# isl-org/Open3D-PointNet2-Semantic3D

Hardware: AMD Instinct MI355X
Metric: points/sec through SA+FP stack (B=16,N=8192) (higher is better)
Workload: dtype f32

## Files before the change

open3d-pointnet2-semantic3d_amd/csrc/pn2_interpolate.hip:

```cpp
#include <math.h>

#include "pn2_common.h"
#include "pn2_three_nn.h"

namespace {

using namespace pn2nn;

PN2_TUNABLE(int, g_nn_blocks, 2048)

template <int kNnChunks>
__global__ void __launch_bounds__(kNnThreads)
three_nn_kernel(int n, int m, const float* __restrict__ xyz1_all, int ld1,
                const float* __restrict__ xyz2_all, float* __restrict__ dist_all,
                int* __restrict__ idx_all) {
    __shared__ __attribute__((aligned(16))) unsigned char slds[kNnWaves * kNnWaveLdsBytes];
    const int wave = __builtin_amdgcn_readfirstlane(threadIdx.x >> 6);
    const int bi = blockIdx.y;
    three_nn_wave<kNnChunks>(n, m, xyz1_all + (size_t)bi * n * ld1, xyz2_all + (size_t)bi * m * 3, dist_all + (size_t)bi * n * 3,
                             idx_all + (size_t)bi * n * 3, blockIdx.x * kNnWaves + wave, gridDim.x * kNnWaves,
                             nn_wave_lds(slds, wave), ld1);
}

template <typename VT, int VEC>
__global__ void __launch_bounds__(256)
three_interpolate_kernel(int m, int c, int n, const float* __restrict__ points_all,
                         const int* __restrict__ idx_all, const float* __restrict__ weight_all,
                         float* __restrict__ out_all) {
    const unsigned cv = (unsigned)c / VEC;
    const unsigned total = (unsigned)n * cv;
    const int bi = blockIdx.y;
    const VT* __restrict__ pts = reinterpret_cast<const VT*>(points_all + (size_t)bi * m * c);
    const int* __restrict__ idx = idx_all + (size_t)bi * n * 3;
    const float* __restrict__ w = weight_all + (size_t)bi * n * 3;
    VT* __restrict__ out = reinterpret_cast<VT*>(out_all + (size_t)bi * n * c);
    for (unsigned e = blockIdx.x * blockDim.x + threadIdx.x; e < total; e += gridDim.x * blockDim.x) {
        const unsigned row = e / cv, col = e - row * cv;
        const int i1 = idx[row * 3 + 0], i2 = idx[row * 3 + 1], i3 = idx[row * 3 + 2];
        const float w1 = w[row * 3 + 0], w2 = w[row * 3 + 1], w3 = w[row * 3 + 2];
        const VT p1 = pts[(size_t)i1 * cv + col], p2 = pts[(size_t)i2 * cv + col], p3 = pts[(size_t)i3 * cv + col];
        out[e] = (p1 * w1 + p2 * w2) + p3 * w3;
    }
}

template <typename VT, int VEC>
__global__ void __launch_bounds__(256)
three_interpolate_grad_kernel(int n, int c, int m, const float* __restrict__ grad_out_all,
                              const int* __restrict__ idx_all, const float* __restrict__ weight_all,
                              float* __restrict__ grad_points_all) {
    const unsigned cv = (unsigned)c / VEC;
    const unsigned total = (unsigned)n * cv;
    const int bi = blockIdx.y;
    const VT* __restrict__ go = reinterpret_cast<const VT*>(grad_out_all + (size_t)bi * n * c);
    const int* __restrict__ idx = idx_all + (size_t)bi * n * 3;
    const float* __restrict__ w = weight_all + (size_t)bi * n * 3;
    float* __restrict__ gp = grad_points_all + (size_t)bi * m * c;
    for (unsigned e = blockIdx.x * blockDim.x + threadIdx.x; e < total; e += gridDim.x * blockDim.x) {
        const unsigned row = e / cv, col = e - row * cv;
        const VT g = go[e];
#pragma unroll
        for (int t = 0; t < 3; ++t) {
            const int ii = idx[row * 3 + t];
            const float wt = w[row * 3 + t];
            float* dst = gp + (size_t)ii * c + col * VEC;
            if constexpr (VEC == 4) {
                atomicAdd(dst + 0, g.x * wt); atomicAdd(dst + 1, g.y * wt);
                atomicAdd(dst + 2, g.z * wt); atomicAdd(dst + 3, g.w * wt);
            } else {
                atomicAdd(dst, g * wt);
            }
        }
    }
}

__global__ void __launch_bounds__(256)
ti_csr_count_kernel(int n3, int m, const int* __restrict__ idx_all, int* __restrict__ cnt_all) {
    const int bi = blockIdx.y;
    const int* __restrict__ idx = idx_all + (size_t)bi * n3;
    int* __restrict__ cnt = cnt_all + (size_t)bi * m;
    for (int e = blockIdx.x * blockDim.x + threadIdx.x; e < n3; e += gridDim.x * blockDim.x) atomicAdd(&cnt[idx[e]], 1);
}

__global__ void __launch_bounds__(256)
ti_csr_scan_kernel(int m, int* __restrict__ cnt_all, int* __restrict__ off_all) {
    __shared__ int part[256];
    const int bi = blockIdx.x, t = threadIdx.x;
    int* __restrict__ cnt = cnt_all + (size_t)bi * m;
    int* __restrict__ off = off_all + (size_t)bi * m;
    const int per = (m + 255) / 256;
    const int lo = t * per < m ? t * per : m, hi = lo + per < m ? lo + per : m;
    int sum = 0;
    for (int i = lo; i < hi; ++i) sum += cnt[i];
    part[t] = sum;
    __syncthreads();
    for (int d = 1; d < 256; d <<= 1) {
        const int v = t >= d ? part[t - d] : 0;
        __syncthreads();
        part[t] += v;
        __syncthreads();
    }
    int run = part[t] - sum;
    for (int i = lo; i < hi; ++i) {
        const int v = cnt[i];
        off[i] = run;
        cnt[i] = 0;
        run += v;
    }
}

__global__ void __launch_bounds__(256)
ti_csr_fill_kernel(int n3, int m, int div, const int* __restrict__ idx_all, const float* __restrict__ weight_all,
                   int weight_kind, const int* __restrict__ off_all, int* __restrict__ cur_all, int* __restrict__ ent_q_all,
                   float* __restrict__ ent_w_all) {
    const int bi = blockIdx.y;
    const int* __restrict__ idx = idx_all + (size_t)bi * n3;
    const float* __restrict__ w = weight_all ? weight_all + (size_t)bi * n3 : nullptr;
    const int* __restrict__ off = off_all + (size_t)bi * m;
    int* __restrict__ cur = cur_all + (size_t)bi * m;
    int* __restrict__ eq = ent_q_all + (size_t)bi * n3;
    float* __restrict__ ew = ent_w_all + (size_t)bi * n3;
    for (int e = blockIdx.x * blockDim.x + threadIdx.x; e < n3; e += gridDim.x * blockDim.x) {
        const int s = idx[e];
        const int p = off[s] + atomicAdd(&cur[s], 1);
        eq[p] = e / div;
        float wt = 1.f;
        if (w && weight_kind == 2) {
            const int r = e / 3, j = e - 3 * r;
            const float r1 = 1.0f / fmaxf(w[r * 3 + 0], 1e-10f), r2 = 1.0f / fmaxf(w[r * 3 + 1], 1e-10f);
            const float r3 = 1.0f / fmaxf(w[r * 3 + 2], 1e-10f);
            const float norm = (r1 + r2) + r3;
            wt = (j == 0 ? r1 : (j == 1 ? r2 : r3)) / norm;
        } else if (w) {
            wt = w[e];
        }
        ew[p] = wt;
    }
}

typedef float f32x4_u __attribute__((ext_vector_type(4), aligned(4)));
template <bool ALIGNED>
__device__ __forceinline__ void ti_csr_gather_body(int bx, int bi, int n, int n3, int c, int stride, int m,
                                                   const float* __restrict__ grad_out_all, const int* __restrict__ off_all,
                                                   const int* __restrict__ ent_q_all, const float* __restrict__ ent_w_all,
                                                   float* __restrict__ grad_points_all, int ostride) {
    const int cv = c >> 2;
    const int spb = 256 / cv;
    const int slot = (int)threadIdx.x / cv, col = (int)threadIdx.x - slot * cv;
    const int s = bx * spb + slot;
    if (slot >= spb || s >= m) return;
    const float* __restrict__ gbase = grad_out_all + (size_t)bi * n * stride + 4 * col;
    auto row4 = [&](int q) -> f32x4 {
        if constexpr (ALIGNED) return *reinterpret_cast<const f32x4*>(gbase + (size_t)q * stride);
        else return *reinterpret_cast<const f32x4_u*>(gbase + (size_t)q * stride);
    };
    const int* __restrict__ off = off_all + (size_t)bi * m;
    const int* __restrict__ eq = ent_q_all + (size_t)bi * n3;
    const float* __restrict__ ew = ent_w_all + (size_t)bi * n3;
    const int lo = off[s], hi = s + 1 < m ? off[s + 1] : n3;
    f32x4 acc = {0.f, 0.f, 0.f, 0.f};
    int e = lo;
    for (; e + 3 < hi; e += 4) {
        int q[4]; float w[4]; f32x4 g[4];
#pragma unroll
        for (int u = 0; u < 4; ++u) { q[u] = eq[e + u]; w[u] = ew[e + u]; }
#pragma unroll
        for (int u = 0; u < 4; ++u) g[u] = row4(q[u]);
#pragma unroll
        for (int u = 0; u < 4; ++u) {
            acc.x = __builtin_fmaf(g[u].x, w[u], acc.x); acc.y = __builtin_fmaf(g[u].y, w[u], acc.y);
            acc.z = __builtin_fmaf(g[u].z, w[u], acc.z); acc.w = __builtin_fmaf(g[u].w, w[u], acc.w);
        }
    }
    for (; e < hi; ++e) {
        const f32x4 g = row4(eq[e]);
        const float w = ew[e];
        acc.x = __builtin_fmaf(g.x, w, acc.x); acc.y = __builtin_fmaf(g.y, w, acc.y);
        acc.z = __builtin_fmaf(g.z, w, acc.z); acc.w = __builtin_fmaf(g.w, w, acc.w);
    }
    reinterpret_cast<f32x4*>(grad_points_all + ((size_t)bi * m + s) * ostride)[col] = acc;
}

template <bool ALIGNED>
__global__ void __launch_bounds__(256)
ti_csr_gather_kernel(int n, int n3, int c, int stride, int m, const float* __restrict__ grad_out_all, const int* __restrict__ off_all,
                     const int* __restrict__ ent_q_all, const float* __restrict__ ent_w_all,
                     float* __restrict__ grad_points_all) {
    ti_csr_gather_body<ALIGNED>((int)blockIdx.x, (int)blockIdx.y, n, n3, c, stride, m, grad_out_all, off_all, ent_q_all, ent_w_all,
                                grad_points_all, c);
}

__global__ void __launch_bounds__(256)
fp_interp_concat_kernel(int n, int m, int c1, int c2, int ostride, int rpw, const float* __restrict__ dist_all,
                        const int* __restrict__ idx_all, const float* __restrict__ points1_all,
                        const float* __restrict__ points2_all, float* __restrict__ out_all) {
    const int lane = threadIdx.x & 63;
    const int wave = __builtin_amdgcn_readfirstlane(threadIdx.x >> 6);
    const int bi = blockIdx.y;
    const int cw = ostride;
    const float* __restrict__ dist = dist_all + (size_t)bi * n * 3;
    const int* __restrict__ idx = idx_all + (size_t)bi * n * 3;
    const float* __restrict__ p2 = points2_all + (size_t)bi * m * c2;
    const float* __restrict__ p1 = points1_all ? points1_all + (size_t)bi * n * c1 : nullptr;
    float* __restrict__ out = out_all + (size_t)bi * n * cw;
    for (int row0 = (blockIdx.x * 4 + wave) * rpw; row0 < n; row0 += gridDim.x * 4 * rpw) {
        int r = row0 + (lane < rpw ? lane : rpw - 1);
        r = r < n ? r : n - 1;
        const float d1 = fmaxf(dist[r * 3 + 0], 1e-10f);
        const float d2 = fmaxf(dist[r * 3 + 1], 1e-10f);
        const float d3 = fmaxf(dist[r * 3 + 2], 1e-10f);
        const float r1 = 1.0f / d1, r2 = 1.0f / d2, r3 = 1.0f / d3;
        const float norm = (r1 + r2) + r3;
        const float w1 = r1 / norm, w2 = r2 / norm, w3 = r3 / norm;
        const int i1 = idx[r * 3 + 0], i2 = idx[r * 3 + 1], i3 = idx[r * 3 + 2];
        const int nrows = n - row0 < rpw ? n - row0 : rpw;
        auto one_row = [&](int rr) {
            const float a1 = __uint_as_float(__builtin_amdgcn_readlane(__float_as_uint(w1), rr));
            const float a2 = __uint_as_float(__builtin_amdgcn_readlane(__float_as_uint(w2), rr));
            const float a3 = __uint_as_float(__builtin_amdgcn_readlane(__float_as_uint(w3), rr));
            const float* __restrict__ s1 = p2 + (size_t)__builtin_amdgcn_readlane(i1, rr) * c2;
            const float* __restrict__ s2 = p2 + (size_t)__builtin_amdgcn_readlane(i2, rr) * c2;
            const float* __restrict__ s3 = p2 + (size_t)__builtin_amdgcn_readlane(i3, rr) * c2;
            float* __restrict__ o = out + (size_t)(row0 + rr) * cw;
#pragma unroll 4
            for (int ch = lane; ch < c2; ch += 64) o[ch] = (s1[ch] * a1 + s2[ch] * a2) + s3[ch] * a3;
            if (p1) {
                const float* __restrict__ q = p1 + (size_t)(row0 + rr) * c1;
                for (int ch = lane; ch < c1; ch += 64) o[c2 + ch] = q[ch];
            }
            if (lane < cw - c1 - c2) o[c1 + c2 + lane] = 0.f;
        };
        int rr = 0;
        for (; rr + 1 < nrows; rr += 2) { one_row(rr); one_row(rr + 1); }
        if (rr < nrows) one_row(rr);
    }
}

template <int CHW, int R>
__global__ void __launch_bounds__(256)
fp_interp_concat_rows_kernel(int n, int m, int c1, int c2, int ostride, int rpw, const float* __restrict__ dist_all,
                             const int* __restrict__ idx_all, const float* __restrict__ points1_all,
                             const float* __restrict__ points2_all, float* __restrict__ out_all) {
    const int lane = threadIdx.x & 63;
    const int wave = __builtin_amdgcn_readfirstlane(threadIdx.x >> 6);
    int bx = blockIdx.x, bi = blockIdx.y;
    {
        const unsigned nwg = gridDim.x * gridDim.y;
        if ((nwg & 7u) == 0u) {
            const unsigned lin = blockIdx.x + gridDim.x * blockIdx.y;
            const unsigned swz = (lin & 7u) * (nwg >> 3) + (lin >> 3);
            bx = (int)(swz % gridDim.x);
            bi = (int)(swz / gridDim.x);
        }
    }
    const int cw = ostride;
    const float* __restrict__ dist = dist_all + (size_t)bi * n * 3;
    const int* __restrict__ idx = idx_all + (size_t)bi * n * 3;
    const float* __restrict__ p2 = points2_all + (size_t)bi * m * c2;
    const float* __restrict__ p1 = points1_all ? points1_all + (size_t)bi * n * c1 : p2;
    float* __restrict__ out = out_all + (size_t)bi * n * cw;
    const int c1m = c1 > 0 ? c1 - 1 : 0;
    for (int row0 = (bx * 4 + wave) * rpw; row0 < n; row0 += gridDim.x * 4 * rpw) {
        int r = row0 + (lane < rpw ? lane : rpw - 1);
        r = r < n ? r : n - 1;
        const float d1 = fmaxf(dist[r * 3 + 0], 1e-10f);
        const float d2 = fmaxf(dist[r * 3 + 1], 1e-10f);
        const float d3 = fmaxf(dist[r * 3 + 2], 1e-10f);
        const float r1 = 1.0f / d1, r2 = 1.0f / d2, r3 = 1.0f / d3;
        const float norm = (r1 + r2) + r3;
        const float w1 = r1 / norm, w2 = r2 / norm, w3 = r3 / norm;
        const int i1 = idx[r * 3 + 0], i2 = idx[r * 3 + 1], i3 = idx[r * 3 + 2];
        const int nrows = n - row0 < rpw ? n - row0 : rpw;
        for (int rr = 0; rr < nrows; rr += R) {
            float v[R][CHW];
#pragma unroll
            for (int q = 0; q < R; ++q) {
                const int rx = rr + q < nrows ? rr + q : nrows - 1;
                const float a1 = __uint_as_float(__builtin_amdgcn_readlane(__float_as_uint(w1), rx));
                const float a2 = __uint_as_float(__builtin_amdgcn_readlane(__float_as_uint(w2), rx));
                const float a3 = __uint_as_float(__builtin_amdgcn_readlane(__float_as_uint(w3), rx));
                const float* __restrict__ s1 = p2 + (size_t)__builtin_amdgcn_readlane(i1, rx) * c2;
                const float* __restrict__ s2 = p2 + (size_t)__builtin_amdgcn_readlane(i2, rx) * c2;
                const float* __restrict__ s3 = p2 + (size_t)__builtin_amdgcn_readlane(i3, rx) * c2;
                const float* __restrict__ qp = p1 + (size_t)(row0 + rx) * c1;
#pragma unroll
                for (int j = 0; j < CHW; ++j) {
                    const int col = lane + 64 * j;
                    const int cc = col < c2 ? col : c2 - 1;
                    int ci = col - c2;
                    ci = ci < 0 ? 0 : (ci > c1m ? c1m : ci);
                    const float x1 = s1[cc], x2 = s2[cc], x3 = s3[cc], xp = qp[ci];
                    const float val = (x1 * a1 + x2 * a2) + x3 * a3;
                    v[q][j] = col < c2 ? val : (col < c2 + c1 ? xp : 0.f);
                }
            }
#pragma unroll
            for (int q = 0; q < R; ++q) {
                if (rr + q < nrows) {
                    float* __restrict__ o = out + (size_t)(row0 + rr + q) * cw;
#pragma unroll
                    for (int j = 0; j < CHW; ++j) {
                        const int col = lane + 64 * j;
                        if (col < cw) o[col] = v[q][j];
                    }
                }
            }
        }
    }
}

template <bool P1V>
__global__ void __launch_bounds__(256)
fp_interp_concat_v4_kernel(int n, int m, int c1, int c2, int ostride, int rpw, int sh2, int sht,
                           const float* __restrict__ dist_all, const int* __restrict__ idx_all,
                           const float* __restrict__ points1_all, const float* __restrict__ points2_all,
                           float* __restrict__ out_all) {
    __shared__ __attribute__((aligned(16))) float swt[4 * 64 * 8];
    const int lane = threadIdx.x & 63;
    const int wave = __builtin_amdgcn_readfirstlane(threadIdx.x >> 6);
    int bx = blockIdx.x, bi = blockIdx.y;
    {
        const unsigned nwg = gridDim.x * gridDim.y;
        if ((nwg & 7u) == 0u) {
            const unsigned lin = blockIdx.x + gridDim.x * blockIdx.y;
            const unsigned swz = (lin & 7u) * (nwg >> 3) + (lin >> 3);
            bx = (int)(swz % gridDim.x);
            bi = (int)(swz / gridDim.x);
        }
    }
    const int cv = ostride >> 2, c2v = c2 >> 2;
    const float* __restrict__ dist = dist_all + (size_t)bi * n * 3;
    const int* __restrict__ idx = idx_all + (size_t)bi * n * 3;
    const f32x4* __restrict__ p2 = reinterpret_cast<const f32x4*>(points2_all + (size_t)bi * m * c2);
    const float* __restrict__ p1 = points1_all ? points1_all + (size_t)bi * n * c1 : nullptr;
    f32x4* __restrict__ out = reinterpret_cast<f32x4*>(out_all + (size_t)bi * n * ostride);
    float* wv = swt + wave * 64 * 8;
    const unsigned m2 = (1u << sh2) - 1u, mt = (1u << sht) - 1u;
    for (int row0 = (bx * 4 + wave) * rpw; row0 < n; row0 += gridDim.x * 4 * rpw) {
        {
            int r = row0 + (lane < rpw ? lane : rpw - 1);
            r = r < n ? r : n - 1;
            const float d1 = fmaxf(dist[r * 3 + 0], 1e-10f);
            const float d2 = fmaxf(dist[r * 3 + 1], 1e-10f);
            const float d3 = fmaxf(dist[r * 3 + 2], 1e-10f);
            const float r1 = 1.0f / d1, r2 = 1.0f / d2, r3 = 1.0f / d3;
            const float norm = (r1 + r2) + r3;
            const f32x4 wq = {r1 / norm, r2 / norm, r3 / norm, 0.f};
            const f32x4 iq = {__int_as_float(idx[r * 3 + 0]), __int_as_float(idx[r * 3 + 1]),
                              __int_as_float(idx[r * 3 + 2]), 0.f};
            *reinterpret_cast<f32x4*>(wv + lane * 8) = wq;
            *reinterpret_cast<f32x4*>(wv + lane * 8 + 4) = iq;
        }
        const int nrows = n - row0 < rpw ? n - row0 : rpw;
        const unsigned E = (unsigned)nrows << sh2;
        for (unsigned e0 = lane; e0 < E; e0 += 64 * 4) {
            f32x4 v[4];
#pragma unroll
            for (int u = 0; u < 4; ++u) {
                unsigned e = e0 + 64 * u;
                e = e < E ? e : E - 1;
                const unsigned row = e >> sh2, col = e & m2;
                const f32x4 wq = *reinterpret_cast<const f32x4*>(wv + row * 8);
                const f32x4 iq = *reinterpret_cast<const f32x4*>(wv + row * 8 + 4);
                const f32x4 x1 = p2[(size_t)__float_as_int(iq[0]) * c2v + col];
                const f32x4 x2 = p2[(size_t)__float_as_int(iq[1]) * c2v + col];
                const f32x4 x3 = p2[(size_t)__float_as_int(iq[2]) * c2v + col];
                v[u] = (x1 * wq[0] + x2 * wq[1]) + x3 * wq[2];
            }
#pragma unroll
            for (int u = 0; u < 4; ++u) {
                const unsigned e = e0 + 64 * u;
                if (e < E) out[(size_t)(row0 + (e >> sh2)) * cv + (e & m2)] = v[u];
            }
        }
        const unsigned ET = (unsigned)nrows << sht;
        for (unsigned e = lane; e < ET; e += 64) {
            const unsigned row = e >> sht, ct = e & mt;
            f32x4 t = {0.f, 0.f, 0.f, 0.f};
            if constexpr (P1V) {
                if ((int)ct * 4 < c1) t = *reinterpret_cast<const f32x4*>(p1 + (size_t)(row0 + row) * c1 + ct * 4);
            } else {
#pragma unroll
                for (int i = 0; i < 4; ++i) {
                    const int ch = (int)ct * 4 + i;
                    if (ch < c1) t[i] = p1[(size_t)(row0 + row) * c1 + ch];
                }
            }
            out[(size_t)(row0 + row) * cv + c2v + ct] = t;
        }
    }
}

inline int grid_x_for(unsigned long long total, int block, int batches) {
    unsigned long long g = (total + block - 1) / block;
    unsigned long long cap = (256ull * 8 + batches - 1) / batches;
    if (cap < 1) cap = 1;
    if (g > cap) g = cap;
    if (g < 1) g = 1;
    return (int)g;
}

}

#ifdef PN2_TUNING_HOOKS
extern "C" int pn2_debug_set_interp(int what, int value) { if (what == 12) { g_nn_blocks = value; return 0; } return -1; }
#endif

extern "C" int pn2_three_nn_ld(int b, int n, int m, const float* xyz1, int ld1, const float* xyz2, float* dist,
                               int* idx, void* stream) {
    if (b <= 0 || n <= 0 || m < 3 || ld1 < 3) return PN2_EINVAL;
    if (!xyz1 || !xyz2 || !dist || !idx) return PN2_ENULL;
    if ((long long)n * ld1 > 0x7fffffffLL || (long long)m * 3 > 0x7fffffffLL || b > 65535) return PN2_ERANGE;
    const int blocks_all = (n + kNnWaves * kNnQ - 1) / (kNnWaves * kNnQ);
    int per = (b * blocks_all + g_nn_blocks - 1) / g_nn_blocks;
    if (per < 1) per = 1;
    dim3 grid((blocks_all + per - 1) / per, b);
    hipStream_t st = static_cast<hipStream_t>(stream);
    if (m <= 64) three_nn_kernel<1><<<grid, kNnThreads, 0, st>>>(n, m, xyz1, ld1, xyz2, dist, idx);
    else if (m <= 256) three_nn_kernel<4><<<grid, kNnThreads, 0, st>>>(n, m, xyz1, ld1, xyz2, dist, idx);
    else three_nn_kernel<16><<<grid, kNnThreads, 0, st>>>(n, m, xyz1, ld1, xyz2, dist, idx);
    PN2_RETURN_IF_LAUNCH_FAILED();
    return PN2_OK;
}

extern "C" int pn2_three_nn(int b, int n, int m, const float* xyz1, const float* xyz2, float* dist,
                            int* idx, void* stream) {
    return pn2_three_nn_ld(b, n, m, xyz1, 3, xyz2, dist, idx, stream);
}

extern "C" int pn2_three_interpolate(int b, int m, int c, int n, const float* points, const int* idx,
                                     const float* weight, float* out, void* stream) {
    if (b <= 0 || m <= 0 || c <= 0 || n <= 0) return PN2_EINVAL;
    if (!points || !idx || !weight || !out) return PN2_ENULL;
    if ((unsigned long long)n * c > 0xffffffffull || b > 65535) return PN2_ERANGE;
    hipStream_t st = static_cast<hipStream_t>(stream);
    const bool vec4 = (c % 4 == 0) && (((uintptr_t)points | (uintptr_t)out) % 16 == 0);
    if (vec4) {
        dim3 grid(grid_x_for((unsigned long long)n * (c / 4), 256, b), b);
        three_interpolate_kernel<f32x4, 4><<<grid, 256, 0, st>>>(m, c, n, points, idx, weight, out);
    } else {
        dim3 grid(grid_x_for((unsigned long long)n * c, 256, b), b);
        three_interpolate_kernel<float, 1><<<grid, 256, 0, st>>>(m, c, n, points, idx, weight, out);
    }
    PN2_RETURN_IF_LAUNCH_FAILED();
    return PN2_OK;
}

extern "C" int pn2_three_interpolate_grad(int b, int n, int c, int m, const float* grad_out,
                                          const int* idx, const float* weight, float* grad_points,
                                          void* stream) {
    if (b <= 0 || m <= 0 || c <= 0 || n <= 0) return PN2_EINVAL;
    if (!grad_out || !idx || !weight || !grad_points) return PN2_ENULL;
    if ((unsigned long long)n * c > 0xffffffffull || b > 65535) return PN2_ERANGE;
    hipStream_t st = static_cast<hipStream_t>(stream);
    hipError_t e = hipMemsetAsync(grad_points, 0, sizeof(float) * (size_t)b * m * c, st);
    if (e != hipSuccess) return (int)e;
    const bool vec4 = (c % 4 == 0) && ((uintptr_t)grad_out % 16 == 0);
    if (vec4) {
        dim3 grid(grid_x_for((unsigned long long)n * (c / 4), 256, b), b);
        three_interpolate_grad_kernel<f32x4, 4><<<grid, 256, 0, st>>>(n, c, m, grad_out, idx, weight, grad_points);
    } else {
        dim3 grid(grid_x_for((unsigned long long)n * c, 256, b), b);
        three_interpolate_grad_kernel<float, 1><<<grid, 256, 0, st>>>(n, c, m, grad_out, idx, weight, grad_points);
    }
    PN2_RETURN_IF_LAUNCH_FAILED();
    return PN2_OK;
}

extern "C" size_t pn2_scatter_plan_bytes(int b, int nent, int nsrc) {
    if (b <= 0 || nent <= 0 || nsrc <= 0) return 0;
    return sizeof(int) * ((size_t)2 * b * nsrc + (size_t)2 * b * nent);
}

extern "C" int pn2_scatter_plan_build(int b, int nent, int div, int nsrc, const int* idx, const float* weight, int weight_kind,
                                      void* plan, size_t plan_bytes, void* stream) {
    if (b <= 0 || nent <= 0 || nsrc <= 0 || div <= 0 || nent % div != 0) return PN2_EINVAL;
    if (weight_kind < 0 || weight_kind > 2 || (weight_kind == 2 && div != 3)) return PN2_EINVAL;
    if (!idx || !plan || (weight_kind != 0 && !weight)) return PN2_ENULL;
    if (b > 65535) return PN2_ERANGE;
    if (plan_bytes < pn2_scatter_plan_bytes(b, nent, nsrc) || ((uintptr_t)plan % 4) != 0) return PN2_EINVAL;
    hipStream_t st = static_cast<hipStream_t>(stream);
    int* cnt = static_cast<int*>(plan);
    int* off = cnt + (size_t)b * nsrc;
    int* ent_q = off + (size_t)b * nsrc;
    float* ent_w = reinterpret_cast<float*>(ent_q + (size_t)b * nent);
    hipError_t e = hipMemsetAsync(cnt, 0, sizeof(int) * (size_t)b * nsrc, st);
    if (e != hipSuccess) return (int)e;
    dim3 ge(grid_x_for((unsigned long long)nent, 256, b), b);
    ti_csr_count_kernel<<<ge, 256, 0, st>>>(nent, nsrc, idx, cnt);
    ti_csr_scan_kernel<<<b, 256, 0, st>>>(nsrc, cnt, off);
    ti_csr_fill_kernel<<<ge, 256, 0, st>>>(nent, nsrc, div, idx, weight_kind ? weight : nullptr, weight_kind, off, cnt, ent_q, ent_w);
    PN2_RETURN_IF_LAUNCH_FAILED();
    return PN2_OK;
}

constexpr int kMaxPlans = 8;
struct PlanDesc {
    int nent, nsrc, div, kind;
    const int* idx;
    const float* w;
    int* cnt;
    int* off;
    int* eq;
    float* ew;
};
struct PlanBatch {
    PlanDesc d[kMaxPlans];
};

__global__ void __launch_bounds__(256)
ti_csr_count_multi_kernel(PlanBatch pb) {
    const PlanDesc& p = pb.d[blockIdx.z];
    const int bi = blockIdx.y;
    const int* __restrict__ idx = p.idx + (size_t)bi * p.nent;
    int* __restrict__ cnt = p.cnt + (size_t)bi * p.nsrc;
    for (int e = blockIdx.x * blockDim.x + threadIdx.x; e < p.nent; e += gridDim.x * blockDim.x) atomicAdd(&cnt[idx[e]], 1);
}

__global__ void __launch_bounds__(256)
ti_csr_scan_multi_kernel(PlanBatch pb) {
    __shared__ int part[256];
    const PlanDesc& p = pb.d[blockIdx.y];
    const int bi = blockIdx.x, t = threadIdx.x, m = p.nsrc;
    int* __restrict__ cnt = p.cnt + (size_t)bi * m;
    int* __restrict__ off = p.off + (size_t)bi * m;
    const int per = (m + 255) / 256;
    const int lo = t * per < m ? t * per : m, hi = lo + per < m ? lo + per : m;
    int sum = 0;
    for (int i = lo; i < hi; ++i) sum += cnt[i];
    part[t] = sum;
    __syncthreads();
    for (int d = 1; d < 256; d <<= 1) {
        const int v = t >= d ? part[t - d] : 0;
        __syncthreads();
        part[t] += v;
        __syncthreads();
    }
    int run = part[t] - sum;
    for (int i = lo; i < hi; ++i) {
        const int v = cnt[i];
        off[i] = run;
        cnt[i] = 0;
        run += v;
    }
}

__global__ void __launch_bounds__(256)
ti_csr_fill_multi_kernel(PlanBatch pb) {
    const PlanDesc& p = pb.d[blockIdx.z];
    const int bi = blockIdx.y, n3 = p.nent, m = p.nsrc;
    const int* __restrict__ idx = p.idx + (size_t)bi * n3;
    const float* __restrict__ w = p.kind ? p.w + (size_t)bi * n3 : nullptr;
    const int* __restrict__ off = p.off + (size_t)bi * m;
    int* __restrict__ cur = p.cnt + (size_t)bi * m;
    int* __restrict__ eq = p.eq + (size_t)bi * n3;
    float* __restrict__ ew = p.ew + (size_t)bi * n3;
    for (int e = blockIdx.x * blockDim.x + threadIdx.x; e < n3; e += gridDim.x * blockDim.x) {
        const int s_ = idx[e];
        const int q = off[s_] + atomicAdd(&cur[s_], 1);
        eq[q] = e / p.div;
        float wt = 1.f;
        if (w && p.kind == 2) {
            const int r = e / 3, j = e - 3 * r;
            const float r1 = 1.0f / fmaxf(w[r * 3 + 0], 1e-10f), r2 = 1.0f / fmaxf(w[r * 3 + 1], 1e-10f);
            const float r3 = 1.0f / fmaxf(w[r * 3 + 2], 1e-10f);
            const float norm = (r1 + r2) + r3;
            wt = (j == 0 ? r1 : (j == 1 ? r2 : r3)) / norm;
        } else if (w) {
            wt = w[e];
        }
        ew[q] = wt;
    }
}

constexpr int kPlanLdsMaxSrc = 16384;
constexpr int kPlanLdsThreads = 1024;
__global__ void __launch_bounds__(kPlanLdsThreads)
ti_csr_build_lds_kernel(PlanBatch pb) {
    extern __shared__ int plan_lds[];
    __shared__ int wsum[kPlanLdsThreads / 64];
    const PlanDesc& p = pb.d[blockIdx.y];
    const int bi = blockIdx.x, t = threadIdx.x, m = p.nsrc, n3 = p.nent;
    int* __restrict__ cnt = plan_lds;
    int* __restrict__ off = plan_lds + m;
    const int* __restrict__ idx = p.idx + (size_t)bi * n3;
    for (int i = t; i < m; i += kPlanLdsThreads) cnt[i] = 0;
    __syncthreads();
    for (int e = t; e < n3; e += kPlanLdsThreads) atomicAdd(&cnt[idx[e]], 1);
    __syncthreads();
    const int per = (m + kPlanLdsThreads - 1) / kPlanLdsThreads;
    const int lo = t * per < m ? t * per : m, hi = lo + per < m ? lo + per : m;
    int sum = 0;
    for (int i = lo; i < hi; ++i) sum += cnt[i];
    int inc = sum;
    const int lane = t & 63, wave = t >> 6;
#pragma unroll
    for (int o = 1; o < 64; o <<= 1) { const int v = __shfl_up(inc, o); if (lane >= o) inc += v; }
    if (lane == 63) wsum[wave] = inc;
    __syncthreads();
    int base = 0;
    for (int w_ = 0; w_ < wave; ++w_) base += wsum[w_];
    int run = base + inc - sum;
    int* __restrict__ gcnt = p.cnt + (size_t)bi * m;
    int* __restrict__ goff = p.off + (size_t)bi * m;
    for (int i = lo; i < hi; ++i) {
        const int v = cnt[i];
        off[i] = run;
        goff[i] = run;
        gcnt[i] = v;
        cnt[i] = 0;
        run += v;
    }
    __syncthreads();
    const float* __restrict__ w = p.kind ? p.w + (size_t)bi * n3 : nullptr;
    int* __restrict__ eq = p.eq + (size_t)bi * n3;
    float* __restrict__ ew = p.ew + (size_t)bi * n3;
    for (int e = t; e < n3; e += kPlanLdsThreads) {
        const int s_ = idx[e];
        const int q = off[s_] + atomicAdd(&cnt[s_], 1);
        eq[q] = e / p.div;
        float wt = 1.f;
        if (w && p.kind == 2) {
            const int r = e / 3, j = e - 3 * r;
            const float r1 = 1.0f / fmaxf(w[r * 3 + 0], 1e-10f), r2 = 1.0f / fmaxf(w[r * 3 + 1], 1e-10f);
            const float r3 = 1.0f / fmaxf(w[r * 3 + 2], 1e-10f);
            const float norm = (r1 + r2) + r3;
            wt = (j == 0 ? r1 : (j == 1 ? r2 : r3)) / norm;
        } else if (w) {
            wt = w[e];
        }
        ew[q] = wt;
    }
}

extern "C" int pn2_scatter_plan_build_multi(int nplans, int b, const int* nent, const int* div, const int* nsrc,
                                            const int* const* idx, const float* const* weight, const int* weight_kind,
                                            void* buffer, const size_t* offset, size_t buffer_bytes, void* stream) {
    if (nplans <= 0 || nplans > kMaxPlans || b <= 0) return PN2_EINVAL;
    if (!nent || !div || !nsrc || !idx || !weight || !weight_kind || !buffer || !offset) return PN2_ENULL;
    if (b > 65535) return PN2_ERANGE;
    PlanBatch pb{};
    int max_ent = 0;
    size_t end = 0;
    for (int i = 0; i < nplans; ++i) {
        if (nent[i] <= 0 || nsrc[i] <= 0 || div[i] <= 0 || nent[i] % div[i] != 0) return PN2_EINVAL;
        if (weight_kind[i] < 0 || weight_kind[i] > 2 || (weight_kind[i] == 2 && div[i] != 3)) return PN2_EINVAL;
        if (!idx[i] || (weight_kind[i] != 0 && !weight[i])) return PN2_ENULL;
        const size_t bytes = pn2_scatter_plan_bytes(b, nent[i], nsrc[i]);
        if (offset[i] % 16 != 0 || offset[i] < end || offset[i] + bytes > buffer_bytes) return PN2_EINVAL;
        end = offset[i] + bytes;
        int* cnt = reinterpret_cast<int*>(static_cast<char*>(buffer) + offset[i]);
        PlanDesc& d = pb.d[i];
        d.nent = nent[i]; d.nsrc = nsrc[i]; d.div = div[i]; d.kind = weight_kind[i];
        d.idx = idx[i]; d.w = weight_kind[i] ? weight[i] : nullptr;
        d.cnt = cnt; d.off = cnt + (size_t)b * nsrc[i]; d.eq = d.off + (size_t)b * nsrc[i];
        d.ew = reinterpret_cast<float*>(d.eq + (size_t)b * nent[i]);
        max_ent = nent[i] > max_ent ? nent[i] : max_ent;
    }
    if (((uintptr_t)buffer % 16) != 0) return PN2_EINVAL;
    hipStream_t st = static_cast<hipStream_t>(stream);
    int max_src = 0;
    for (int i = 0; i < nplans; ++i) max_src = nsrc[i] > max_src ? nsrc[i] : max_src;
    if (max_src <= kPlanLdsMaxSrc) {
        const size_t lds = sizeof(int) * 2 * (size_t)max_src;
        if (int e = pn2_allow_lds<ti_csr_build_lds_kernel>(sizeof(int) * 2 * kPlanLdsMaxSrc)) return e;
        ti_csr_build_lds_kernel<<<dim3(b, nplans), kPlanLdsThreads, lds, st>>>(pb);
        PN2_RETURN_IF_LAUNCH_FAILED();
        return PN2_OK;
    }
    hipError_t e = hipMemsetAsync(static_cast<char*>(buffer) + offset[0], 0, end - offset[0], st);
    if (e != hipSuccess) return (int)e;
    dim3 ge(grid_x_for((unsigned long long)max_ent, 256, b * nplans), b, nplans);
    ti_csr_count_multi_kernel<<<ge, 256, 0, st>>>(pb);
    ti_csr_scan_multi_kernel<<<dim3(b, nplans), 256, 0, st>>>(pb);
    ti_csr_fill_multi_kernel<<<ge, 256, 0, st>>>(pb);
    PN2_RETURN_IF_LAUNCH_FAILED();
    return PN2_OK;
}

extern "C" int pn2_scatter_plan_apply(int b, int nent, int div, int c, int nsrc, const float* rows_in, int in_stride,
                                      const void* plan, size_t plan_bytes, float* out, void* stream) {
    if (b <= 0 || nent <= 0 || nsrc <= 0 || div <= 0 || nent % div != 0 || c <= 0 || in_stride < c) return PN2_EINVAL;
    if (!rows_in || !plan || !out) return PN2_ENULL;
    if (c % 4 != 0 || c > 1024 || ((uintptr_t)out % 16) != 0 || ((uintptr_t)rows_in % 4) != 0) return PN2_EUNSUP;
    if (b > 65535) return PN2_ERANGE;
    if (plan_bytes < pn2_scatter_plan_bytes(b, nent, nsrc) || ((uintptr_t)plan % 4) != 0) return PN2_EINVAL;
    hipStream_t st = static_cast<hipStream_t>(stream);
    const int* off = static_cast<const int*>(plan) + (size_t)b * nsrc;
    const int* ent_q = off + (size_t)b * nsrc;
    const float* ent_w = reinterpret_cast<const float*>(ent_q + (size_t)b * nent);
    const int spb = 256 / (c / 4);
    dim3 gg((nsrc + spb - 1) / spb, b);
    const bool aligned = ((uintptr_t)rows_in % 16) == 0 && in_stride % 4 == 0;
    if (aligned) ti_csr_gather_kernel<true><<<gg, 256, 0, st>>>(nent / div, nent, c, in_stride, nsrc, rows_in, off, ent_q, ent_w, out);
    else ti_csr_gather_kernel<false><<<gg, 256, 0, st>>>(nent / div, nent, c, in_stride, nsrc, rows_in, off, ent_q, ent_w, out);
    PN2_RETURN_IF_LAUNCH_FAILED();
    return PN2_OK;
}

constexpr int kMaxApplyPlans = 4;
struct ApplyDesc {
    int n, n3, c, stride, aligned;
    const float* rows_in;
    const int* off;
    const int* eq;
    const float* ew;
    float* out;
};
struct ApplyBatch {
    ApplyDesc d[kMaxApplyPlans];
    int start[kMaxApplyPlans + 1];
    int nsrc, ostride;
};

__global__ void __launch_bounds__(256)
ti_csr_gather_multi_kernel(ApplyBatch ab) {
    const int bx0 = blockIdx.x;
    int pi = 0;
#pragma unroll
    for (int k = 1; k < kMaxApplyPlans; ++k) pi += bx0 >= ab.start[k] ? 1 : 0;
    const ApplyDesc& d = ab.d[pi];
    const int bx = bx0 - ab.start[pi];
    if (d.aligned) ti_csr_gather_body<true>(bx, (int)blockIdx.y, d.n, d.n3, d.c, d.stride, ab.nsrc, d.rows_in, d.off, d.eq, d.ew, d.out, ab.ostride);
// ... 123 lines not shown
```

open3d-pointnet2-semantic3d_amd/csrc/pn2_three_nn.h:

```cpp
#pragma once
#include <math.h>

#include "pn2_common.h"

namespace pn2nn {

typedef float f32x4 __attribute__((ext_vector_type(4)));

constexpr int kNnThreads = 256;
constexpr int kNnWaves = kNnThreads / 64;
constexpr int kNnQ = 8;
constexpr int kNnList = 32;

struct NnPoint { float x, y, z; };

__device__ __forceinline__ int nn_wave_imax(int v) {
    asm volatile(
        "s_nop 1\n"
        "v_max_i32_dpp %0, %0, %0 row_shr:1 row_mask:0xf bank_mask:0xf\n s_nop 1\n"
        "v_max_i32_dpp %0, %0, %0 row_shr:2 row_mask:0xf bank_mask:0xf\n s_nop 1\n"
        "v_max_i32_dpp %0, %0, %0 row_shr:4 row_mask:0xf bank_mask:0xf\n s_nop 1\n"
        "v_max_i32_dpp %0, %0, %0 row_shr:8 row_mask:0xf bank_mask:0xf\n s_nop 1\n"
        "v_max_i32_dpp %0, %0, %0 row_bcast:15 row_mask:0xa bank_mask:0xf\n s_nop 1\n"
        "v_max_i32_dpp %0, %0, %0 row_bcast:31 row_mask:0xc bank_mask:0xf\n s_nop 1\n"
        : "+v"(v));
    return __builtin_amdgcn_readlane(v, 63);
}

__device__ __forceinline__ float nn_fmin(float a, float b) {
    float r;
    asm("v_min_f32 %0, %1, %2" : "=v"(r) : "v"(a), "v"(b));
    return r;
}
__device__ __forceinline__ float nn_fmin3(float a, float b, float c) {
    float r;
    asm("v_min3_f32 %0, %1, %2, %3" : "=v"(r) : "v"(a), "v"(b), "v"(c));
    return r;
}

#ifndef PN2_NN_STAGES
#define PN2_NN_STAGES 9
#endif

template <int CTRL>
__device__ __forceinline__ float nn_dpp(float v) {
    return __int_as_float(__builtin_amdgcn_update_dpp(0, __float_as_int(v), CTRL, 0xf, 0xf, true));
}

__device__ __forceinline__ void nn_merge3(float& t0, float& t1, float& t2, float b0, float b1, float b2) {
    const float r0 = fminf(t0, b0);
    const float r1 = fminf(fminf(t1, b1), fmaxf(t0, b0));
    const float r2 = fminf(fminf(fminf(t2, b2), fmaxf(t0, b1)), fmaxf(t1, b0));
    t0 = r0; t1 = r1; t2 = r2;
}

struct NnWaveLds {
    int* wl;
    double* wd;
    float* wm;
    float* wq;
    float* wr;
    int* wc;
};
constexpr int kNnWaveLdsBytes = kNnQ * kNnList * 12 + kNnQ * 64 * 4 + kNnQ * 4 * 8 + kNnQ * 4;
__device__ __forceinline__ NnWaveLds nn_wave_lds(unsigned char* base, int w) {
    unsigned char* p = base + (size_t)w * kNnWaveLdsBytes;
    NnWaveLds s;
    s.wd = reinterpret_cast<double*>(p);                  p += kNnQ * kNnList * 8;
    s.wm = reinterpret_cast<float*>(p);                   p += kNnQ * 64 * 4;
    s.wq = reinterpret_cast<float*>(p);                   p += kNnQ * 4 * 4;
    s.wr = reinterpret_cast<float*>(p);                   p += kNnQ * 4 * 4;
    s.wl = reinterpret_cast<int*>(p);                     p += kNnQ * kNnList * 4;
    s.wc = reinterpret_cast<int*>(p);
    return s;
}

template <int kNnChunks>
__device__ __forceinline__ void three_nn_wave(int n, int m, const float* __restrict__ xyz1, const float* __restrict__ xyz2,
                                              float* __restrict__ dist_all, int* __restrict__ idx_all, int grp, int gstride,
                                              const NnWaveLds& S, int ld1 = 3) {
    const int lane = threadIdx.x & 63;
    const int ngroups = (n + kNnQ - 1) / kNnQ;
    if (grp >= ngroups) return;
    const NnPoint* __restrict__ cand = reinterpret_cast<const NnPoint*>(xyz2);
    int* wl = S.wl;
    double* wd = S.wd;
    float* wm = S.wm;
    float* wq = S.wq;
    float* wr = S.wr;
    int* wc = S.wc;

    const float ox = xyz2[0], oy = xyz2[1], oz = xyz2[2];
    const int last = m - 1;
    const int nblk = (m + 64 * kNnChunks - 1) / (64 * kNnChunks);
    float cx[kNnChunks], cy[kNnChunks], cz[kNnChunks], cc[kNnChunks];
    float rc = 0.f;
    auto load_block = [&](int blk) {
#pragma unroll
        for (int t = 0; t < kNnChunks; ++t) {
            const int k = (blk * kNnChunks + t) * 64 + lane;
            const NnPoint p = cand[k < last ? k : last];
            const float x = p.x - ox, y = p.y - oy, z = p.z - oz;
            cx[t] = x; cy[t] = y; cz[t] = z;
            cc[t] = __builtin_fmaf(z, z, __builtin_fmaf(y, y, x * x));
            rc = fmaxf(rc, fmaxf(fabsf(x), fmaxf(fabsf(y), fabsf(z))));
        }
    };
    auto load_queries = [&](int g) {
        const int l = lane < 3 * kNnQ ? lane : 3 * kNnQ - 1;
        int jq = g * kNnQ + l / 3;
        jq = jq < n ? jq : n - 1;
        return xyz1[jq * ld1 + l % 3];
    };
    float qnext = load_queries(grp);
    if (nblk == 1) load_block(0);
  for (; grp < ngroups; grp += gstride) {
    const int q0 = grp * kNnQ;
    const float qv = qnext;
    if (grp + gstride < ngroups) qnext = load_queries(grp + gstride);
    float ax[kNnQ], ay[kNnQ], az[kNnQ];
    float rq = 0.f;
#pragma unroll
    for (int q = 0; q < kNnQ; ++q) {
        const float rx = __uint_as_float(__builtin_amdgcn_readlane(__float_as_uint(qv), 3 * q + 0));
        const float ry = __uint_as_float(__builtin_amdgcn_readlane(__float_as_uint(qv), 3 * q + 1));
        const float rz = __uint_as_float(__builtin_amdgcn_readlane(__float_as_uint(qv), 3 * q + 2));
        if (lane == 0) *reinterpret_cast<f32x4*>(wr + q * 4) = f32x4{rx, ry, rz, 0.f};
        const float x = rx - ox, y = ry - oy, z = rz - oz;
        ax[q] = -2.0f * x; ay[q] = -2.0f * y; az[q] = -2.0f * z;
        rq = fmaxf(rq, fmaxf(fabsf(x), fmaxf(fabsf(y), fabsf(z))));
    }
    auto rank = [&](int q, int t) {
        return __builtin_fmaf(ax[q], cx[t], __builtin_fmaf(ay[q], cy[t], __builtin_fmaf(az[q], cz[t], cc[t])));
    };

    float mn[kNnQ];
#pragma unroll
    for (int q = 0; q < kNnQ; ++q) mn[q] = INFINITY;
    for (int blk = 0; blk < nblk; ++blk) {
        if (nblk > 1) load_block(blk);
        auto one_chunk = [&](int t) {
            const int k = (blk * kNnChunks + t) * 64 + lane;
            const int cbase = (blk * kNnChunks + t) * 64;
            if (cbase + 64 <= m) {
#pragma unroll
                for (int q = 0; q < kNnQ; ++q) mn[q] = nn_fmin(mn[q], rank(q, t));
            } else if (cbase < m) {
                const bool valid = k < m;
#pragma unroll
                for (int q = 0; q < kNnQ; ++q) mn[q] = nn_fmin(mn[q], valid ? rank(q, t) : INFINITY);
            }
        };
        if constexpr (kNnChunks >= 2) {
#pragma unroll
            for (int t = 0; t < kNnChunks; t += 2) {
                if ((blk * kNnChunks + t + 2) * 64 <= m) {
#pragma unroll
                    for (int q = 0; q < kNnQ; ++q) mn[q] = nn_fmin3(mn[q], rank(q, t), rank(q, t + 1));
                } else {
                    one_chunk(t);
                    one_chunk(t + 1);
                }
            }
        } else {
            one_chunk(0);
        }
    }
    if constexpr (PN2_NN_STAGES < 2) {
        float acc = 0.f;
#pragma unroll
        for (int q = 0; q < kNnQ; ++q) acc += mn[q];
        if (acc == 12345.f) dist_all[lane] = acc;
        continue;
    }
    const float R = fmaxf(__int_as_float(nn_wave_imax(__float_as_int(rc))), rq);
    const float E3 = R * R * (3.0f * 64.0f * 5.9604645e-8f * 1.001f);
#pragma unroll
    for (int q = 0; q < kNnQ; ++q) wm[q * 64 + lane] = mn[q];
    float t0, t1, t2;
    {
        const int g = lane >> 3, part = lane & 7;
        const f32x4 v0 = *reinterpret_cast<const f32x4*>(wm + g * 64 + part * 8);
        const f32x4 v1 = *reinterpret_cast<const f32x4*>(wm + g * 64 + part * 8 + 4);
        t0 = fminf(fminf(v0[0], v0[1]), v0[2]);
        t2 = fmaxf(fmaxf(v0[0], v0[1]), v0[2]);
        t1 = __builtin_amdgcn_fmed3f(v0[0], v0[1], v0[2]);
        const float rest[5] = {v0[3], v1[0], v1[1], v1[2], v1[3]};
#pragma unroll
        for (int i = 0; i < 5; ++i) {
            const float d = rest[i];
            const float n0 = fminf(t0, d);
            const float n1 = __builtin_amdgcn_fmed3f(t0, t1, d);
            const float n2 = __builtin_amdgcn_fmed3f(t1, t2, d);
            t0 = n0; t1 = n1; t2 = n2;
        }
        nn_merge3(t0, t1, t2, nn_dpp<0xB1>(t0), nn_dpp<0xB1>(t1), nn_dpp<0xB1>(t2));
        nn_merge3(t0, t1, t2, nn_dpp<0x4E>(t0), nn_dpp<0x4E>(t1), nn_dpp<0x4E>(t2));
        nn_merge3(t0, t1, t2, nn_dpp<0x141>(t0), nn_dpp<0x141>(t1), nn_dpp<0x141>(t2));
    }
    float thr[kNnQ];
#pragma unroll
    for (int q = 0; q < kNnQ; ++q)
        thr[q] = __uint_as_float(__builtin_amdgcn_readlane(__float_as_uint(t2), q * 8)) + E3;

    if constexpr (PN2_NN_STAGES < 3) {
        float acc = 0.f;
#pragma unroll
        for (int q = 0; q < kNnQ; ++q) acc += thr[q];
        if (acc == 12345.f) dist_all[lane] = acc;
        continue;
    }
#pragma unroll
    for (int q = 0; q < kNnQ; ++q) {
        if (lane == 0) {
            *reinterpret_cast<f32x4*>(wq + q * 4) = f32x4{ax[q], ay[q], az[q], thr[q]};
            wc[q] = 0;
        }
    }
    unsigned todo = 0u;
#pragma unroll
    for (int q = 0; q < kNnQ; ++q) todo |= (mn[q] <= thr[q] ? 1u : 0u) << q;
    for (int blk = 0; blk < nblk; ++blk) {
        if (nblk > 1) load_block(blk);
        int nvalid = (m - lane - blk * kNnChunks * 64 + 63) >> 6;
        nvalid = nvalid < 0 ? 0 : (nvalid > kNnChunks ? kNnChunks : nvalid);
        const unsigned vmask = (1u << nvalid) - 1u;
        unsigned td = todo;
        while (td != 0u) {
            const int q = __ffs(td) - 1;
            td &= td - 1u;
            const f32x4 qp = *reinterpret_cast<const f32x4*>(wq + q * 4);
            unsigned hm = 0u;
#pragma unroll
            for (int t = 0; t < kNnChunks; ++t) {
                const float sv = __builtin_fmaf(qp[0], cx[t], __builtin_fmaf(qp[1], cy[t], __builtin_fmaf(qp[2], cz[t], cc[t])));
                hm |= (sv <= qp[3] ? 1u : 0u) << t;
            }
            hm &= vmask;
            while (hm != 0u) {
                const int t = __ffs(hm) - 1;
                hm &= hm - 1u;
                const int kk = (blk * kNnChunks + t) * 64 + lane;
                const int pos = atomicAdd(&wc[q], 1);
                if (pos < kNnList) wl[q * kNnList + pos] = kk;
            }
        }
    }
    int cnt[kNnQ];
#pragma unroll
    for (int q = 0; q < kNnQ; ++q) cnt[q] = __builtin_amdgcn_readfirstlane(wc[q]);

    if constexpr (PN2_NN_STAGES < 4) {
        int acc = 0;
#pragma unroll
        for (int q = 0; q < kNnQ; ++q) acc += cnt[q];
        if (acc == 12345) idx_all[lane] = acc + wl[lane];
        continue;
    }
    {
        const int g = lane >> 3, part = lane & 7;
        int cg = 0;
#pragma unroll
        for (int q = 0; q < kNnQ; ++q) cg = g == q ? cnt[q] : cg;
        if (q0 + g < n) {
            const size_t o = (size_t)(q0 + g) * 3;
            if (cg <= kNnList) {
                const double qx = (double)wr[g * 4 + 0], qy = (double)wr[g * 4 + 1], qz = (double)wr[g * 4 + 2];
                for (int e = part; e < cg; e += 8) {
                    const int kk = wl[g * kNnList + e];
                    const double dx = qx - (double)xyz2[kk * 3 + 0];
                    const double dy = qy - (double)xyz2[kk * 3 + 1];
                    const double dz = qz - (double)xyz2[kk * 3 + 2];
                    wd[g * kNnList + e] = (dx * dx + dy * dy) + dz * dz;
                }
                for (int e = part; e < cg; e += 8) {
                    const double d = wd[g * kNnList + e];
                    const int kk = wl[g * kNnList + e];
                    int rank = 0;
                    for (int j0 = 0; j0 < cg; j0 += 8) {
                        double dj[8];
                        int kj[8];
#pragma unroll
                        for (int u = 0; u < 8; ++u) { dj[u] = wd[g * kNnList + j0 + u]; kj[u] = wl[g * kNnList + j0 + u]; }
#pragma unroll
                        for (int u = 0; u < 8; ++u)
                            rank += (j0 + u < cg && (dj[u] < d || (dj[u] == d && kj[u] < kk))) ? 1 : 0;
                    }
                    if (rank < 3) { dist_all[o + rank] = (float)d; idx_all[o + rank] = kk; }
                }
            } else if (part == 0) {
                const int jq = q0 + g;
                const double dqx = xyz1[jq * ld1 + 0], dqy = xyz1[jq * ld1 + 1], dqz = xyz1[jq * ld1 + 2];
                double b1 = INFINITY, b2 = INFINITY, b3 = INFINITY;
                int i1 = 0, i2 = 0, i3 = 0;
                for (int kk = 0; kk < m; ++kk) {
                    const double dx = dqx - (double)xyz2[kk * 3 + 0];
                    const double dy = dqy - (double)xyz2[kk * 3 + 1];
                    const double dz = dqz - (double)xyz2[kk * 3 + 2];
                    const double d = (dx * dx + dy * dy) + dz * dz;
                    if (d < b3) {
                        if (d < b1) { b3 = b2; i3 = i2; b2 = b1; i2 = i1; b1 = d; i1 = kk; }
                        else if (d < b2) { b3 = b2; i3 = i2; b2 = d; i2 = kk; }
                        else { b3 = d; i3 = kk; }
                    }
                }
                dist_all[o + 0] = (float)b1; dist_all[o + 1] = (float)b2; dist_all[o + 2] = (float)b3;
                idx_all[o + 0] = i1; idx_all[o + 1] = i2; idx_all[o + 2] = i3;
            }
        }
    }
  }
}

}
```

Before: 382.7 million.

## Add wave-wide ballot-based candidate collection for three_nn with m up to 1024

For 256 < m <= 1024, the kernel now stages the centered candidate points and their squared norms into shared LDS once per block, loaded cooperatively by all waves with a block barrier. The second pass, which gathers candidates under each query's threshold, then runs across the whole wave: each round deals 4 candidate lanes times 16 chunks per query and compacts hits with ballot/mbcnt. This replaces the per-query serial loops and LDS atomics. The cost is extra LDS per block, which may lower occupancy, plus a __syncthreads and more divergent rounds when many lanes pass the prefilter.

```diff
diff --git a/open3d-pointnet2-semantic3d_amd/csrc/pn2_interpolate.hip b/open3d-pointnet2-semantic3d_amd/csrc/pn2_interpolate.hip
--- a/open3d-pointnet2-semantic3d_amd/csrc/pn2_interpolate.hip
+++ b/open3d-pointnet2-semantic3d_amd/csrc/pn2_interpolate.hip
@@ -9,17 +9,18 @@
 
 PN2_TUNABLE(int, g_nn_blocks, 2048)
 
-template <int kNnChunks>
+template <int kNnChunks, bool kWide>
 __global__ void __launch_bounds__(kNnThreads)
 three_nn_kernel(int n, int m, const float* __restrict__ xyz1_all, int ld1,
                 const float* __restrict__ xyz2_all, float* __restrict__ dist_all,
                 int* __restrict__ idx_all) {
-    __shared__ __attribute__((aligned(16))) unsigned char slds[kNnWaves * kNnWaveLdsBytes];
+    __shared__ __attribute__((aligned(16))) unsigned char slds[kNnWaves * kNnWaveLdsBytes + (kWide ? kNnStageBytes<kNnChunks> : 0)];
     const int wave = __builtin_amdgcn_readfirstlane(threadIdx.x >> 6);
     const int bi = blockIdx.y;
-    three_nn_wave<kNnChunks>(n, m, xyz1_all + (size_t)bi * n * ld1, xyz2_all + (size_t)bi * m * 3, dist_all + (size_t)bi * n * 3,
-                             idx_all + (size_t)bi * n * 3, blockIdx.x * kNnWaves + wave, gridDim.x * kNnWaves,
-                             nn_wave_lds(slds, wave), ld1);
+    three_nn_wave<kNnChunks, kWide>(n, m, xyz1_all + (size_t)bi * n * ld1, xyz2_all + (size_t)bi * m * 3,
+                                    dist_all + (size_t)bi * n * 3, idx_all + (size_t)bi * n * 3, blockIdx.x * kNnWaves + wave,
+                                    gridDim.x * kNnWaves, nn_wave_lds(slds, wave), ld1,
+                                    reinterpret_cast<f32x4*>(slds + kNnWaves * kNnWaveLdsBytes));
 }
 
 template <typename VT, int VEC>
@@ -415,9 +416,10 @@
     if (per < 1) per = 1;
     dim3 grid((blocks_all + per - 1) / per, b);
     hipStream_t st = static_cast<hipStream_t>(stream);
-    if (m <= 64) three_nn_kernel<1><<<grid, kNnThreads, 0, st>>>(n, m, xyz1, ld1, xyz2, dist, idx);
-    else if (m <= 256) three_nn_kernel<4><<<grid, kNnThreads, 0, st>>>(n, m, xyz1, ld1, xyz2, dist, idx);
-    else three_nn_kernel<16><<<grid, kNnThreads, 0, st>>>(n, m, xyz1, ld1, xyz2, dist, idx);
+    if (m <= 64) three_nn_kernel<1, false><<<grid, kNnThreads, 0, st>>>(n, m, xyz1, ld1, xyz2, dist, idx);
+    else if (m <= 256) three_nn_kernel<4, false><<<grid, kNnThreads, 0, st>>>(n, m, xyz1, ld1, xyz2, dist, idx);
+    else if (m <= 64 * 16) three_nn_kernel<16, true><<<grid, kNnThreads, 0, st>>>(n, m, xyz1, ld1, xyz2, dist, idx);
+    else three_nn_kernel<16, false><<<grid, kNnThreads, 0, st>>>(n, m, xyz1, ld1, xyz2, dist, idx);
     PN2_RETURN_IF_LAUNCH_FAILED();
     return PN2_OK;
 }
diff --git a/open3d-pointnet2-semantic3d_amd/csrc/pn2_three_nn.h b/open3d-pointnet2-semantic3d_amd/csrc/pn2_three_nn.h
--- a/open3d-pointnet2-semantic3d_amd/csrc/pn2_three_nn.h
+++ b/open3d-pointnet2-semantic3d_amd/csrc/pn2_three_nn.h
@@ -63,6 +63,8 @@
     int* wc;
 };
 constexpr int kNnWaveLdsBytes = kNnQ * kNnList * 12 + kNnQ * 64 * 4 + kNnQ * 4 * 8 + kNnQ * 4;
+template <int kNnChunks>
+constexpr int kNnStageBytes = 64 * (kNnChunks + 1) * 16;
 __device__ __forceinline__ NnWaveLds nn_wave_lds(unsigned char* base, int w) {
     unsigned char* p = base + (size_t)w * kNnWaveLdsBytes;
     NnWaveLds s;
@@ -75,13 +77,17 @@
     return s;
 }
 
-template <int kNnChunks>
+template <int kNnChunks, bool kWide = false>
 __device__ __forceinline__ void three_nn_wave(int n, int m, const float* __restrict__ xyz1, const float* __restrict__ xyz2,
                                               float* __restrict__ dist_all, int* __restrict__ idx_all, int grp, int gstride,
-                                              const NnWaveLds& S, int ld1 = 3) {
+                                              const NnWaveLds& S, int ld1 = 3,
+                                              f32x4* stage = nullptr) {
+    static_assert(!kWide || kNnChunks == 16, "the wave-wide pass 2 deals 4 pairs x 16 chunks per round");
     const int lane = threadIdx.x & 63;
     const int ngroups = (n + kNnQ - 1) / kNnQ;
-    if (grp >= ngroups) return;
+    if constexpr (!kWide) {
+        if (grp >= ngroups) return;
+    }
     const NnPoint* __restrict__ cand = reinterpret_cast<const NnPoint*>(xyz2);
     int* wl = S.wl;
     double* wd = S.wd;
@@ -112,8 +118,28 @@
         jq = jq < n ? jq : n - 1;
         return xyz1[jq * ld1 + l % 3];
     };
-    float qnext = load_queries(grp);
-    if (nblk == 1) load_block(0);
+    float qnext = load_queries(grp < ngroups ? grp : ngroups - 1);
+    if constexpr (kWide) {
+        const int w = __builtin_amdgcn_readfirstlane(threadIdx.x >> 6) & (kNnWaves - 1);
+#pragma unroll
+        for (int u = 0; u < kNnChunks / kNnWaves; ++u) {
+            const int t = u * kNnWaves + w;
+            const int k = t * 64 + lane;
+            const NnPoint p = cand[k < last ? k : last];
+            const float x = p.x - ox, y = p.y - oy, z = p.z - oz;
+            stage[lane * (kNnChunks + 1) + t] = f32x4{x, y, z, __builtin_fmaf(z, z, __builtin_fmaf(y, y, x * x))};
+        }
+        __syncthreads();
+        if (grp >= ngroups) return;
+#pragma unroll
+        for (int t = 0; t < kNnChunks; ++t) {
+            const f32x4 v = stage[lane * (kNnChunks + 1) + t];
+            cx[t] = v[0]; cy[t] = v[1]; cz[t] = v[2]; cc[t] = v[3];
+            rc = fmaxf(rc, fmaxf(fabsf(v[0]), fmaxf(fabsf(v[1]), fabsf(v[2]))));
+        }
+    } else {
+        if (nblk == 1) load_block(0);
+    }
   for (; grp < ngroups; grp += gstride) {
     const int q0 = grp * kNnQ;
     const float qv = qnext;
@@ -210,45 +236,83 @@
         if (acc == 12345.f) dist_all[lane] = acc;
         continue;
     }
-#pragma unroll
-    for (int q = 0; q < kNnQ; ++q) {
-        if (lane == 0) {
-            *reinterpret_cast<f32x4*>(wq + q * 4) = f32x4{ax[q], ay[q], az[q], thr[q]};
-            wc[q] = 0;
-        }
-    }
-    unsigned todo = 0u;
-#pragma unroll
-    for (int q = 0; q < kNnQ; ++q) todo |= (mn[q] <= thr[q] ? 1u : 0u) << q;
-    for (int blk = 0; blk < nblk; ++blk) {
-        if (nblk > 1) load_block(blk);
-        int nvalid = (m - lane - blk * kNnChunks * 64 + 63) >> 6;
-        nvalid = nvalid < 0 ? 0 : (nvalid > kNnChunks ? kNnChunks : nvalid);
-        const unsigned vmask = (1u << nvalid) - 1u;
-        unsigned td = todo;
-        while (td != 0u) {
-            const int q = __ffs(td) - 1;
-            td &= td - 1u;
-            const f32x4 qp = *reinterpret_cast<const f32x4*>(wq + q * 4);
-            unsigned hm = 0u;
-#pragma unroll
-            for (int t = 0; t < kNnChunks; ++t) {
-                const float sv = __builtin_fmaf(qp[0], cx[t], __builtin_fmaf(qp[1], cy[t], __builtin_fmaf(qp[2], cz[t], cc[t])));
-                hm |= (sv <= qp[3] ? 1u : 0u) << t;
-            }
-            hm &= vmask;
-            while (hm != 0u) {
-                const int t = __ffs(hm) - 1;
-                hm &= hm - 1u;
-                const int kk = (blk * kNnChunks + t) * 64 + lane;
-                const int pos = atomicAdd(&wc[q], 1);
-                if (pos < kNnList) wl[q * kNnList + pos] = kk;
-            }
-        }
-    }
     int cnt[kNnQ];
-#pragma unroll
-    for (int q = 0; q < kNnQ; ++q) cnt[q] = __builtin_amdgcn_readfirstlane(wc[q]);
+    if constexpr (kWide) {
+        unsigned char* pl = reinterpret_cast<unsigned char*>(wm);
+        int np[kNnQ];
+        int npmax = 0;
+#pragma unroll
+        for (int q = 0; q < kNnQ; ++q) {
+            const bool in = mn[q] <= thr[q];
+            const unsigned long long mk = __ballot(in);
+            np[q] = __popcll(mk);
+            npmax = np[q] > npmax ? np[q] : npmax;
+            cnt[q] = 0;
+            const int pos = (int)__builtin_amdgcn_mbcnt_hi((unsigned)(mk >> 32), __builtin_amdgcn_mbcnt_lo((unsigned)mk, 0u));
+            if (in) pl[q * 64 + pos] = (unsigned char)lane;
+        }
+        const int tw = lane & 15;
+        const int jw = lane >> 4;
+        const f32x4* srow = stage + tw;
+        auto one_round = [&](int q, int j0) {
+            const int j = j0 + jw;
+            const int src = (int)pl[q * 64 + (j & 63)] & 63;
+            const f32x4 cv = srow[src * (kNnChunks + 1)];
+            const float sv = __builtin_fmaf(ax[q], cv[0], __builtin_fmaf(ay[q], cv[1], __builtin_fmaf(az[q], cv[2], cv[3])));
+            const int kk = tw * 64 + src;
+            const bool hit = j < np[q] && kk < m && sv <= thr[q];
+            const unsigned long long hb = __ballot(hit);
+            const int pos = cnt[q] + (int)__builtin_amdgcn_mbcnt_hi((unsigned)(hb >> 32), __builtin_amdgcn_mbcnt_lo((unsigned)hb, 0u));
+            if (hit && pos < kNnList) wl[q * kNnList + pos] = kk;
+            cnt[q] += __popcll(hb);
+        };
+#pragma unroll
+        for (int q = 0; q < kNnQ; ++q) one_round(q, 0);
+        for (int j0 = 4; j0 < npmax; j0 += 4) {
+#pragma unroll
+            for (int q = 0; q < kNnQ; ++q)
+                if (j0 < np[q]) one_round(q, j0);
+        }
+    } else {
+#pragma unroll
+        for (int q = 0; q < kNnQ; ++q) {
+            if (lane == 0) {
+                *reinterpret_cast<f32x4*>(wq + q * 4) = f32x4{ax[q], ay[q], az[q], thr[q]};
+                wc[q] = 0;
+            }
+        }
+        unsigned todo = 0u;
+#pragma unroll
+        for (int q = 0; q < kNnQ; ++q) todo |= (mn[q] <= thr[q] ? 1u : 0u) << q;
+        for (int blk = 0; blk < nblk; ++blk) {
+            if (nblk > 1) load_block(blk);
+            int nvalid = (m - lane - blk * kNnChunks * 64 + 63) >> 6;
+            nvalid = nvalid < 0 ? 0 : (nvalid > kNnChunks ? kNnChunks : nvalid);
+            const unsigned vmask = (1u << nvalid) - 1u;
+            unsigned td = todo;
+            while (td != 0u) {
+                const int q = __ffs(td) - 1;
+                td &= td - 1u;
+                const f32x4 qp = *reinterpret_cast<const f32x4*>(wq + q * 4);
+                unsigned hm = 0u;
+#pragma unroll
+                for (int t = 0; t < kNnChunks; ++t) {
+                    const float sv = __builtin_fmaf(qp[0], cx[t], __builtin_fmaf(qp[1], cy[t], __builtin_fmaf(qp[2], cz[t], cc[t])));
+                    hm |= (sv <= qp[3] ? 1u : 0u) << t;
+                }
+                hm &= vmask;
+                while (hm != 0u) {
+                    const int t = __ffs(hm) - 1;
+                    hm &= hm - 1u;
+                    const int kk = (blk * kNnChunks + t) * 64 + lane;
+                    const int pos = atomicAdd(&wc[q], 1);
+                    if (pos < kNnList) wl[q * kNnList + pos] = kk;
+                }
+            }
+        }
+#pragma unroll
+        for (int q = 0; q < kNnQ; ++q) cnt[q] = __builtin_amdgcn_readfirstlane(wc[q]);
+    }
 
     if constexpr (PN2_NN_STAGES < 4) {
         int acc = 0;
```

Measured after the change: 384.2 million, median of 6. Within noise of the previous version (+0.4%).
